# DeadAt0m/ActiveSparseShifts-PyTorch

Hardware: AMD Instinct MI355X
Metric: Gelem/s, Shift2d fwd+bwd N64/C256/224x224 (higher is better)
Workload: dtype f32; 1 GPU; Shift2d SSL fwd+bwd N64 C256 224x224 fp32, padding 0, per GPU; batch sharded over 1 GPU(s), no collectives

## Files before the change

### activesparseshifts-pytorch_amd/csrc/shiftnd_cl_tiled.hip

```cpp
#include "shiftnd_common.hpp"
#include "shiftnd_launch.hpp"

namespace shiftnd {
namespace {

constexpr int kR = 3;
constexpr int kTW = 32;
constexpr int kLine = 128;
constexpr int kPW = kTW + 2 * kR;
constexpr int kRing = 2 * kR + 1;
constexpr int kPitch = kLine / 4 + 1;
constexpr int kRowWords = kPW * kPitch;
constexpr int kPieces = kPW * (kLine / 16);
constexpr int kNP = (kPieces + kThreads - 1) / kThreads;
#ifndef CLT_DEPTH
#define CLT_DEPTH 3
#endif

struct ClTiledParams {
    const char *x;
    char *out;
    const void *w;
    int64_t wzp;
    uint32_t fill;
// ... 221 lines not shown
        if (hs + kR < H) store_row(hs + kR, pv);
        __syncthreads();
        load_row(hs + kDepth + kR, ylast, pv);
        const uint32_t so = static_cast<uint32_t>(h - h0) * ostep;
        int rowb[NSH];
#pragma unroll
        for (int k = 0; k < NSH; ++k) {
            const int sy = fold_once(hs - ssh[k]);
            const uint32_t r = static_cast<uint32_t>(sy & ~(sy >> 31));
            const uint32_t sl = r - __umulhi(r, 613566757u) * kRing;
            rowb[k] = (16 + static_cast<int>(sl) * (kRowWords * 4)) | ((sy >> 31) & kNeg);
        }
        uint32_t v[4];
#pragma unroll
        for (int i = 0; i < 4; ++i) {
            v[i] = 0;
#pragma unroll
            for (int j = 0; j < NE; ++j) {
                const uint32_t e = *reinterpret_cast<const EL *>(ringz + max(rowb[OUT_CL ? j : i] + xoff[i][j], 0));
                v[i] |= e << (8 * ES * j);
            }
        }
#pragma unroll
        for (int i = 0; i < 4; ++i) __builtin_amdgcn_raw_buffer_store_b32(v[i], ores, ooff[i], so, 0);
    };
    int hb = h0;
    for (; hb + kDepth <= h1; hb += kDepth) {
#pragma unroll
        for (int d = 0; d < kDepth; ++d) step(hb + d, pvs[d]);
    }
#pragma unroll
    for (int d = 0; d < kDepth - 1; ++d)
        if (hb + d < h1) step(hb + d, pvs[d]);

    const bool wrap_rows = periodic && (h0 + LH < kR || h1 + LH > H - kR);
    if (far || (wrap_rows && ring_ok)) {
        asm volatile("s_waitcnt vmcnt(0)" ::: "memory");
#pragma unroll
        for (int i = 0; i < 4; ++i) {
#pragma unroll
            for (int j = 0; j < NE; ++j) {
                const bool all_rows = (far >> (4 * i + j)) & 1u;
                if (!all_rows && !(wrap_rows && ((ring_ok >> (4 * i + j)) & 1u))) continue;
                const int D = static_cast<int>(threadIdx.x) + kThreads * i;
                const int ch = OUT_CL ? lane_a * NE + j : D / RD;
                const int col = OUT_CL ? lane_b + 8 * i : (D % RD) * NE + j;
                const EL *xe = reinterpret_cast<const EL *>(xn);
                EL *o = reinterpret_cast<EL *>(on) + (OUT_CL ? ((static_cast<int64_t>(dz) * OH + h0) * OW + w0 + col) * C + c0 + ch
                                                             : ((static_cast<int64_t>(c0 + ch) * OD + dz) * OH + h0) * OW + w0 + col);
                const int64_t zoff = ND3 ? static_cast<int64_t>(tab_pz[ch]) * H * W * C : 0;
                const int shc = csh[OUT_CL ? j : i], shs = ssh[OUT_CL ? j : i];
                for (int h = h0; h < h1; ++h) {
                    const int sy = H == 1 ? 0 : fold_index(h + LH - shc, H, p.pad);
                    if (all_rows || h + LH - shs < 0 || h + LH - shs >= H)
                        *o = sy >= 0 ? xe[zoff + (static_cast<int64_t>(sy) * W + gcol[i][j]) * C + c0 + ch] : static_cast<EL>(p.fill);
                    o += OUT_CL ? OW * C : OW;
                }
            }
        }
    }
}

constexpr int kBTW = 16;
constexpr int kBPW = kBTW + 2 * kR + 1;
constexpr int kBRing = 8;
constexpr int kBPieces = kBPW * (kLine / 16);
static_assert(kBPieces <= kThreads, "one piece of each tensor per thread");

struct ClTiledBwdParams {
    const char *x, *go;
    char *gx;
    const void *w;
    double *partials;
    int wkind, N, C, H, W, pad;
    int OH, OW, LH, LW;
    int go_nchw;
    int go_pieces;
    int wtiles, cblocks, bands, band_rows;
    unsigned xcd_blocks;
    FastDiv d_wtiles, d_cblocks, d_bands;
    FastDiv d_perH, d_perW, d_perOH, d_perOW;
};

template <typename T, bool ACTIVE, bool GO_NCHW, int TW = kBTW>
__global__ __launch_bounds__(kThreads) void cl_tiled_backward(const ClTiledBwdParams p) {
    static_assert(TW == kBTW || !GO_NCHW, "the wide strip takes a channels-last gradient");
    constexpr int BPW = TW + 2 * kR + 1;
    constexpr int BPIECES = BPW * (kLine / 16);
    constexpr int NPX = (BPIECES + kThreads - 1) / kThreads;
    typedef uint32_t u4 __attribute__((ext_vector_type(4)));
    using S = typename T::S;
    using CT = typename T::C;
    static_assert(sizeof(S) == 4 || sizeof(S) == 2, "fp32, fp16, bf16");
    constexpr int ES = sizeof(S), CB = kLine / ES;
    constexpr int PL = kThreads / CB, NI = TW / PL;
    constexpr int PITCHX = kLine / 4, PITCHG = GO_NCHW ? kPitch : kLine / 4;
    constexpr int BROWX = BPW * PITCHX, BROWG = BPW * PITCHG, BRINGX = kBRing * BROWX, BRINGG = kBRing * BROWG;
    __shared__ __attribute__((aligned(16))) uint32_t ring_all[4 + BRINGX + BRINGG + 4];
    uint32_t *const ring = ring_all + 4;
    constexpr int kDump = BRINGX + BRINGG;
    constexpr int kNeg = -(1 << 24);
    if (threadIdx.x < 4) ring_all[threadIdx.x] = 0u;

    unsigned b = p.xcd_blocks ? (blockIdx.x & 7u) * p.xcd_blocks + (blockIdx.x >> 3) : blockIdx.x;
    const int cb = static_cast<int>(b - fdiv(b, p.d_cblocks) * p.cblocks);
    b = fdiv(b, p.d_cblocks);
    const int pidx = static_cast<int>(b);
    const int wt = static_cast<int>(b - fdiv(b, p.d_wtiles) * p.wtiles);
    b = fdiv(b, p.d_wtiles);
    const int band = static_cast<int>(b - fdiv(b, p.d_bands) * p.bands);
    const int n = static_cast<int>(fdiv(b, p.d_bands));
    const int w0 = wt * TW, c0 = cb * CB;
    const int h0 = band * p.band_rows, h1 = min(p.H, h0 + p.band_rows);
    const int H = p.H, W = p.W, C = p.C, OH = p.OH, OW = p.OW, LH = p.LH, LW = p.LW;
    const int64_t img = static_cast<int64_t>(n) * H * W * C * ES;
    const char *xn = p.x + img, *gn = p.go + static_cast<int64_t>(n) * OH * OW * C * ES;
    char *on = p.gx + img;
    const uint32_t img_bytes = static_cast<uint32_t>(H) * static_cast<uint32_t>(W) * static_cast<uint32_t>(C) * ES;
    const uint32_t go_bytes = static_cast<uint32_t>(OH) * static_cast<uint32_t>(OW) * static_cast<uint32_t>(C) * ES;
    const __amdgpu_buffer_rsrc_t xres = __builtin_amdgcn_make_buffer_rsrc(const_cast<char *>(xn), 0, img_bytes, kBufferFlags);
    const __amdgpu_buffer_rsrc_t gres = __builtin_amdgcn_make_buffer_rsrc(const_cast<char *>(gn), 0, go_bytes, kBufferFlags);
    const __amdgpu_buffer_rsrc_t ores = __builtin_amdgcn_make_buffer_rsrc(on, 0, img_bytes, kBufferFlags);
    auto g_index = [&](int ch, int r, int cc) {
        return GO_NCHW ? (static_cast<int64_t>(ch) * OH + r) * OW + cc : (static_cast<int64_t>(r) * OW + cc) * C + ch;
    };

    const int q = static_cast<int>(threadIdx.x);
    uint32_t poff[NPX], poffg[NPX];
    int pdst[NPX];
#pragma unroll
    for (int k = 0; k < NPX; ++k) {
        const int qk = q + k * kThreads;
        const bool piece = qk < BPIECES;
        const int px = qk >> 3, part = qk & 7, gxs = w0 - kR + px;
        poff[k] = (piece && gxs >= 0 && gxs < W && c0 * ES + part * 16 < C * ES) ? static_cast<uint32_t>(gxs) * C * ES + c0 * ES + part * 16 : kOutOfRange;
        poffg[k] = (piece && gxs >= LW && gxs < LW + OW && c0 * ES + part * 16 < C * ES) ? static_cast<uint32_t>(gxs - LW) * C * ES + c0 * ES + part * 16 : kOutOfRange;
        pdst[k] = piece ? px * PITCHX + part * 4 : -1;
    }
    const uint32_t row_bytes = static_cast<uint32_t>(W) * C * ES;
    constexpr int kDepth = CLT_DEPTH;
    constexpr int kGE = CB * BPW, kGN = GO_NCHW ? (kGE + kThreads - 1) / kThreads : 1;
    struct GRow {
        u4 v[NPX];
        uint32_t e[kGN];
    };
    uint32_t goff[kGN];
    int gdst[kGN];
    if constexpr (GO_NCHW) {
#pragma unroll
        for (int k = 0; k < kGN; ++k) {
            const int e = k * kThreads + q, ch = e / BPW, pxe = e - ch * BPW, gxe = w0 - kR + pxe;
            const bool ok = e < kGE && gxe >= LW && gxe < LW + OW && c0 + ch < C;
            goff[k] = ok ? (static_cast<uint32_t>(c0 + ch) * OH * OW + (gxe - LW)) * ES : kOutOfRange;
            gdst[k] = e < kGE ? pxe * (PITCHG * 4) + ch * ES : -1;
        }
    }
    constexpr int kGPC = 7;
    const bool g_pieces = GO_NCHW && ES == 4 && p.go_pieces != 0;
    uint32_t gpoff = kOutOfRange;
    int gpdst[4] = {-1, -1, -1, -1};
    if constexpr (GO_NCHW && ES == 4) {
        const int ch = q / kGPC, pi = q - ch * kGPC;
        const int cstart = w0 - kR - LW;
        const int e0 = ((cstart >> 2) + pi) * 4;
        const bool ok = q < CB * kGPC && e0 >= 0 && e0 < OW && c0 + ch < C;
        gpoff = ok ? (static_cast<uint32_t>(c0 + ch) * OH * OW + e0) * ES : kOutOfRange;
#pragma unroll
        for (int j = 0; j < 4; ++j) {
            const int pxj = e0 + j - cstart;
            gpdst[j] = (q < CB * kGPC && pxj >= 0 && pxj < BPW) ? pxj * (PITCHG * 4) + ch * ES : -1;
        }
    }
    const uint32_t grow_bytes = static_cast<uint32_t>(OW) * (GO_NCHW ? 1 : C) * ES;
    struct XRow {
        u4 v[NPX];
    };
    XRow pvx[kDepth];
    GRow pvg[kDepth];
    auto load_row = [&](int y, int ylast, XRow &vx, GRow &vg) {
        const int unwanted = (y >> 31) | ((ylast - y) >> 31);
        const uint32_t so = static_cast<uint32_t>(y & ~unwanted) * row_bytes, dead = static_cast<uint32_t>(unwanted) & kOutOfRange;
#pragma unroll
        for (int k = 0; k < NPX; ++k) vx.v[k] = __builtin_amdgcn_raw_buffer_load_b128(xres, poff[k] | dead, so, 0);
        const int unwanted_g = unwanted | ((y - LH) >> 31) | ((LH + OH - 1 - y) >> 31);
        const uint32_t sg = static_cast<uint32_t>((y - LH) & ~unwanted_g) * grow_bytes, dead_g = static_cast<uint32_t>(unwanted_g) & kOutOfRange;
        if constexpr (GO_NCHW) {
            if (g_pieces) {
                vg.v[0] = __builtin_amdgcn_raw_buffer_load_b128(gres, gpoff | dead_g, sg, 0);
            } else {
#pragma unroll
                for (int k = 0; k < kGN; ++k) {
                    if constexpr (ES == 4) vg.e[k] = __builtin_amdgcn_raw_buffer_load_b32(gres, goff[k] | dead_g, sg, 0);
                    else vg.e[k] = __builtin_amdgcn_raw_buffer_load_b16(gres, goff[k] | dead_g, sg, 0);
                }
            }
        } else {
#pragma unroll
            for (int k = 0; k < NPX; ++k) vg.v[k] = __builtin_amdgcn_raw_buffer_load_b128(gres, poffg[k] | dead_g, sg, 0);
        }
    };
    auto store_row = [&](int y, const XRow &vx, const GRow &vg) {
        const int slot = y & (kBRing - 1);
#pragma unroll
        for (int k = 0; k < NPX; ++k) {
            uint32_t *dx = ring + (pdst[k] >= 0 ? slot * BROWX + pdst[k] : kDump);
            *reinterpret_cast<u4 *>(__builtin_assume_aligned(dx, 16)) = vx.v[k];
        }
        if constexpr (GO_NCHW) {
            char *gbase = reinterpret_cast<char *>(ring) + (BRINGX + slot * BROWG) * 4;
            char *dump = reinterpret_cast<char *>(ring) + kDump * 4;
            if (g_pieces) {
                const uint32_t ge[4] = {vg.v[0].x, vg.v[0].y, vg.v[0].z, vg.v[0].w};
#pragma unroll
                for (int j = 0; j < 4; ++j) *reinterpret_cast<uint32_t *>(gpdst[j] >= 0 ? gbase + gpdst[j] : dump) = ge[j];
            } else {
#pragma unroll
                for (int k = 0; k < kGN; ++k) {
                    char *d = gdst[k] >= 0 ? gbase + gdst[k] : dump;
                    if constexpr (ES == 4) *reinterpret_cast<uint32_t *>(d) = vg.e[k];
                    else *reinterpret_cast<uint16_t *>(d) = static_cast<uint16_t>(vg.e[k]);
                }
            }
        } else {
#pragma unroll
            for (int k = 0; k < NPX; ++k) {
                uint32_t *dg = ring + (pdst[k] >= 0 ? BRINGX + slot * BROWG + pdst[k] : kDump);
                *reinterpret_cast<u4 *>(__builtin_assume_aligned(dg, 16)) = vg.v[k];
            }
        }
    };
    const int ylast = min(H - 1, h1 + kR);
    XRow prex[2 * kR + 1];
    GRow preg[2 * kR + 1];
#pragma unroll
    for (int d = 0; d < kDepth; ++d) load_row(h0 + kR + 1 + d, ylast, pvx[d], pvg[d]);
#pragma unroll
    for (int r = 0; r <= 2 * kR; ++r) load_row(h0 - kR + r, ylast, prex[r], preg[r]);

    const int lane_a = static_cast<int>(threadIdx.x) % CB, lane_b = static_cast<int>(threadIdx.x) / CB;
    const int c = c0 + lane_a;
    const bool live_c = c < C;
    int64_t sh[3] = {0, 0, 0};
    CT dw[3] = {CT(0), CT(0), CT(0)};
    {
        const int wcol[3] = {-1, 0, 1};
        CT wv[3];
        load_weights3<CT>(p.w, p.wkind, static_cast<int64_t>(live_c ? c : C - 1) * 2, wcol, wv);
        prep_shift_backward<CT>(wv[1], ACTIVE, sh[1], dw[0]);
        prep_shift_backward<CT>(wv[2], ACTIVE, sh[2], dw[1]);
    }
    const int csxH = canon_shift(sh[1], H, p.pad, p.d_perH), csxW = canon_shift(sh[2], W, p.pad, p.d_perW);
    const int csgH = canon_shift(ACTIVE ? sh[1] : -sh[1], OH, p.pad, p.d_perOH), csgW = canon_shift(ACTIVE ? sh[2] : -sh[2], OW, p.pad, p.d_perOW);
    const int perH = map_period(H, p.pad), perW = map_period(W, p.pad), perOH = map_period(OH, p.pad), perOW = map_period(OW, p.pad);
    const int sh_s = (perH && 2 * csxH > perH) ? csxH - perH : csxH, sw_s = (perW && 2 * csxW > perW) ? csxW - perW : csxW;
    const int gh_s = (perOH && 2 * csgH > perOH) ? csgH - perOH : csgH, gw_s = (perOW && 2 * csgW > perOW) ? csgW - perOW : csgW;
    const bool in_ring = sh_s >= -kR && sh_s <= kR && sw_s >= -kR && sw_s <= kR && gh_s >= -kR && gh_s <= kR && gw_s >= -kR && gw_s <= kR;
    const bool near_c = live_c && in_ring, far_c = live_c && !in_ring;
    auto fold_h = [&](int idx) { return H == 1 ? 0 : fold_index(idx, H, p.pad); };
    auto fold_w = [&](int idx) { return W == 1 ? 0 : fold_index(idx, W, p.pad); };
    auto fold_gh = [&](int idx) { const int r = OH == 1 ? 0 : fold_index(idx, OH, p.pad); return r < 0 ? -1 : r + LH; };
    auto fold_gw = [&](int idx) { const int r = OW == 1 ? 0 : fold_index(idx, OW, p.pad); return r < 0 ? -1 : r + LW; };
    int xc0[NI], xc1[NI], gc0[NI], gc1[NI], gd[NI];
    uint32_t ooff[NI];
    bool live[NI], scol[NI], cpass[NI];
    int lcount[NI];
#pragma unroll
    for (int i = 0; i < NI; ++i) {
        const int col = lane_b + PL * i, wq = w0 + min(col, W - 1 - w0);
        cpass[i] = wq >= LW && wq < LW + OW;
        const int a0 = cpass[i] ? fold_w(wq - csxW) : -1, a1 = cpass[i] ? fold_w(wq - csxW + 1) : -1;
        const int b0 = cpass[i] ? fold_gw(wq - LW - csgW) : -1, b1 = (ACTIVE && cpass[i]) ? fold_gw(wq - LW - csgW + 1) : -1;
        auto outside = [&](int sx) { return sx >= 0 && (sx < w0 - kR || sx > w0 + TW + kR); };
        scol[i] = near_c && w0 + col < W && (outside(a0) || outside(a1) || outside(b0) || outside(b1));
        live[i] = near_c && w0 + col < W && !scol[i];
        lcount[i] = (live[i] && cpass[i]) ? -1 : 0;
        auto lds_col = [&](int sx, int pitch) { return (live[i] && sx >= 0) ? (sx - (w0 - kR)) * (pitch * 4) + lane_a * ES : kNeg; };
        xc0[i] = lds_col(a0, PITCHX);
        xc1[i] = lds_col(a1, PITCHX);
        gc0[i] = lds_col(b0, PITCHG);
        gc1[i] = lds_col(b1, PITCHG);
        gd[i] = (col + kR) * (PITCHG * 4) + lane_a * ES;
        ooff[i] = live[i] ? (static_cast<uint32_t>(h0 * W + w0 + col) * C + c) * ES : kOutOfRange;
    }
    const uint32_t ostep = static_cast<uint32_t>(W) * C * ES;

#pragma unroll
    for (int r = 0; r <= 2 * kR; ++r) {
        const int y = h0 - kR + r;
        if (y >= 0 && y < H) store_row(y, prex[r], preg[r]);
    }
    const char *ringz = reinterpret_cast<const char *>(ring_all);
    constexpr int ringx = 16, ringg = 16 + BRINGX * 4;
    double acc[2] = {0.0, 0.0};
    auto lds_s = [&](int base, int row, int colo) {
        return *reinterpret_cast<const S *>(ringz + max(base + row + colo, 0));
    };
    auto lds_f = [&](int base, int row, int colo) { return widen<T>(lds_s(base, row, colo)); };
    auto row_off = [&](int sy) { return ((sy & (kBRing - 1)) * (BROWX * 4)) | ((sy >> 31) & kNeg); };
    auto row_off_g = [&](int sy) { return ((sy & (kBRing - 1)) * (BROWG * 4)) | ((sy >> 31) & kNeg); };
    const int fm = (p.pad == 3 || p.pad == 4) ? -1 : 0;
    const int fLo = p.pad == 4 ? -1 : 0, fHi = p.pad == 1 ? H - 1 : (p.pad == 3 ? 2 * H - 2 : 2 * H - 1);
    const int zneg = p.pad == 0 ? kNeg : 0;
    auto fold_once = [&](int idx, int n, int lo_c, int hi_c) {
        const int below = idx >> 31, above = (n - 1 - idx) >> 31, t = idx & fm;
        const int r = (idx & ~(below | above)) | ((lo_c - t) & below) | ((hi_c - t) & above) | ((below | above) & zneg);
        return n == 1 ? 0 : r;
    };
    auto fold1 = [&](int idx) { return fold_once(idx, H, fLo, fHi); };
    const int gLo = p.pad == 4 ? -1 : 0, gHi = p.pad == 1 ? OH - 1 : (p.pad == 3 ? 2 * OH - 2 : 2 * OH - 1);
    auto fold1g = [&](int idx) { return fold_once(idx, OH, gLo, gHi) + LH; };
    const bool srow = near_c && p.pad == 3 && H > 1 && sh_s == -kR && h1 == H;
    const bool srow_g = ACTIVE && near_c && p.pad == 3 && OH > 1 && gh_s == -kR;
    const bool periodic = p.pad == 2 && H > 1;
    auto wraps = [&](int h) {
        const int g0 = h - LH - gh_s;
        const bool in_rows = h >= LH && h < LH + OH;
        return periodic && near_c && (h - sh_s < 0 || h + 1 - sh_s >= H || (in_rows && OH > 1 && (g0 < 0 || g0 + (ACTIVE ? 1 : 0) >= OH)));
    };
    int xrow1 = fold1(h0 - sh_s);
    int grow1 = fold1g(h0 - LH - gh_s);
    auto step = [&](int h, XRow &vx, GRow &vg) {
        __syncthreads();
        if (h + kR + 1 < H) store_row(h + kR + 1, vx, vg);
        __syncthreads();
        load_row(h + kDepth + kR + 1, ylast, vx, vg);
        const uint32_t so = static_cast<uint32_t>(h - h0) * ostep;
        const int xr0 = row_off(xrow1);
        xrow1 = fold1(h + 1 - sh_s);
        const int xr1 = row_off(xrow1);
        const bool rpass = h >= LH && h < LH + OH;
        int gr0, gr1 = kNeg;
        if constexpr (ACTIVE) {
            gr0 = rpass ? row_off_g(grow1) : kNeg;
            grow1 = fold1g(h + 1 - LH - gh_s);
            gr1 = rpass ? row_off_g(grow1) : kNeg;
        } else {
            gr0 = rpass ? row_off_g(fold1g(h - LH - gh_s)) : kNeg;
        }
        const int gdr = (h & (kBRing - 1)) * (BROWG * 4);
        int skip = 0;
        if (p.pad == 3) skip = ((srow && h == H - 1) || (srow_g && h == LH + OH - 1)) ? -1 : 0;
        else if (p.pad == 2) skip = wraps(h) ? -1 : 0;
        const int stepok = (rpass ? -1 : 0) & ~skip;
        S res[NI];
        CT s0 = CT(0), s1 = CT(0);
#pragma unroll
        for (int i = 0; i < NI; ++i) {
            CT v[4], wg[3];
            v[0] = lds_f(ringx, xr0, xc0[i]);
            v[1] = lds_f(ringx, xr1, xc0[i]);
            v[2] = lds_f(ringx, xr0, xc1[i]);
            v[3] = lds_f(ringx, xr1, xc1[i]);
            const CT graw = widen<T>(*reinterpret_cast<const S *>(ringz + ringg + gdr + gd[i]));
            const uint32_t counted = static_cast<uint32_t>(lcount[i] & stepok);
            weight_grads_nd<2, CT>(v, dw, wg);
            static_assert(sizeof(CT) == 4, "fp32 compute type");
            s0 += __builtin_bit_cast(CT, __builtin_bit_cast(uint32_t, graw * wg[0]) & counted);
            s1 += __builtin_bit_cast(CT, __builtin_bit_cast(uint32_t, graw * wg[1]) & counted);
            if constexpr (ACTIVE) {
                v[0] = lds_f(ringg, gr0, gc0[i]);
                v[1] = lds_f(ringg, gr1, gc0[i]);
                v[2] = lds_f(ringg, gr0, gc1[i]);
                v[3] = lds_f(ringg, gr1, gc1[i]);
                res[i] = narrow<T>(interp_t<T, 2>(v, dw));
            } else {
                res[i] = lds_s(ringg, gr0, gc0[i]);
            }
        }
        acc[0] += static_cast<double>(s0);
        acc[1] += static_cast<double>(s1);
#pragma unroll
        for (int i = 0; i < NI; ++i) {
            if constexpr (ES == 4) {
                uint32_t bits;
                __builtin_memcpy(&bits, &res[i], 4);
                __builtin_amdgcn_raw_buffer_store_b32(bits, ores, ooff[i] | (static_cast<uint32_t>(skip) & kOutOfRange), so, 0);
            } else {
                uint16_t bits;
                __builtin_memcpy(&bits, &res[i], 2);
                __builtin_amdgcn_raw_buffer_store_b16(bits, ores, ooff[i] | (static_cast<uint32_t>(skip) & kOutOfRange), so, 0);
            }
        }
    };
    int hb = h0;
    for (; hb + kDepth <= h1; hb += kDepth) {
#pragma unroll
        for (int d = 0; d < kDepth; ++d) step(hb + d, pvx[d], pvg[d]);
    }
#pragma unroll
    for (int d = 0; d < kDepth - 1; ++d)
        if (hb + d < h1) step(hb + d, pvx[d], pvg[d]);

    auto far_element = [&](int ch, int h, int wq, int cxH, int cxW, int cgH, int cgW, const CT (&fr)[3], double &t0, double &t1) {
        const S *xe = reinterpret_cast<const S *>(xn) + ch, *ge = reinterpret_cast<const S *>(gn);
        S *oe = reinterpret_cast<S *>(on) + ch;
        auto tap_s = [&](const S *base, int r, int cc) { return (r >= 0 && cc >= 0) ? base[(static_cast<int64_t>(r) * W + cc) * C] : narrow<T>(CT(0)); };
        auto tap = [&](const S *base, int r, int cc) { return widen<T>(tap_s(base, r, cc)); };
        auto gtap_s = [&](int r, int cc) { return (r >= 0 && cc >= 0) ? ge[g_index(ch, r, cc)] : narrow<T>(CT(0)); };
        auto gtap = [&](int r, int cc) { return widen<T>(gtap_s(r, cc)); };
        if (!(h >= LH && h < LH + OH && wq >= LW && wq < LW + OW)) {
            oe[(static_cast<int64_t>(h) * W + wq) * C] = narrow<T>(CT(0));
            return;
        }
        const int a0 = fold_w(wq - cxW), a1 = fold_w(wq - cxW + 1);
        const int b0 = fold_gw(wq - LW - cgW) - LW, b1 = fold_gw(wq - LW - cgW + 1) - LW;
        const int r0 = fold_h(h - cxH), r1 = fold_h(h - cxH + 1);
        const int s0 = fold_gh(h - LH - cgH) - LH, s1 = fold_gh(h - LH - cgH + 1) - LH;
        CT v[4] = {tap(xe, r0, a0), tap(xe, r1, a0), tap(xe, r0, a1), tap(xe, r1, a1)}, wg[3];
        const CT gval = widen<T>(ge[g_index(ch, h - LH, wq - LW)]);
        weight_grads_nd<2, CT>(v, fr, wg);
        t0 += static_cast<double>(gval * wg[0]);
        t1 += static_cast<double>(gval * wg[1]);
        S r;
        if constexpr (ACTIVE) {
            CT u[4] = {gtap(s0, b0), gtap(s1, b0), gtap(s0, b1), gtap(s1, b1)};
            r = narrow<T>(interp_t<T, 2>(u, fr));
        } else {
            r = gtap_s(s0, b0);
        }
        oe[(static_cast<int64_t>(h) * W + wq) * C] = r;
    };
    bool any_scol = false;
#pragma unroll
    for (int i = 0; i < NI; ++i) any_scol = any_scol || scol[i];
    const bool wrap_rows = periodic && near_c && (h0 <= kR || h1 >= H - kR - 1 || (h0 <= LH + kR && h1 > LH) || (h1 >= LH + OH - kR - 1 && h0 < LH + OH));
    if (near_c && (any_scol || srow || srow_g || wrap_rows)) {
#pragma unroll
        for (int i = 0; i < NI; ++i) {
            const int wq = w0 + lane_b + PL * i;
            if (wq >= W) continue;
            for (int h = h0; h < h1; ++h) {
                if (!(scol[i] || (srow && h == H - 1) || (srow_g && h == LH + OH - 1) || wraps(h))) continue;
                far_element(c, h, wq, csxH, csxW, csgH, csgW, dw, acc[0], acc[1]);
            }
        }
    }
    {
        __shared__ unsigned long long far_mask_s;
        __syncthreads();
        if (threadIdx.x < 64) {
            const unsigned long long m = __ballot(far_c && static_cast<int>(threadIdx.x) < CB);
            if (threadIdx.x == 0) far_mask_s = m;
        }
        __syncthreads();
        unsigned long long fm_left = far_mask_s;
        double *fred = reinterpret_cast<double *>(ring_all);
        while (fm_left) {
            const int fch = __builtin_ctzll(fm_left);
            fm_left &= fm_left - 1;
            const int cf = c0 + fch;
            int64_t fsh[3] = {0, 0, 0};
            CT ffr[3] = {CT(0), CT(0), CT(0)};
            {
                const int wcol[3] = {-1, 0, 1};
                CT wv[3];
                load_weights3<CT>(p.w, p.wkind, static_cast<int64_t>(cf) * 2, wcol, wv);
                prep_shift_backward<CT>(wv[1], ACTIVE, fsh[1], ffr[0]);
                prep_shift_backward<CT>(wv[2], ACTIVE, fsh[2], ffr[1]);
            }
            const int fxH = canon_shift(fsh[1], H, p.pad, p.d_perH), fxW = canon_shift(fsh[2], W, p.pad, p.d_perW);
            const int fgH = canon_shift(ACTIVE ? fsh[1] : -fsh[1], OH, p.pad, p.d_perOH), fgW = canon_shift(ACTIVE ? fsh[2] : -fsh[2], OW, p.pad, p.d_perOW);
            double t0 = 0.0, t1 = 0.0;
            const int nelem = (h1 - h0) * TW;
            for (int q = static_cast<int>(threadIdx.x); q < nelem; q += kThreads) {
                const int h = h0 + q / TW, wq = w0 + q % TW;
                if (wq < W) far_element(cf, h, wq, fxH, fxW, fgH, fgW, ffr, t0, t1);
            }
            __syncthreads();
            fred[threadIdx.x * 2] = t0;
            fred[threadIdx.x * 2 + 1] = t1;
            __syncthreads();
            if (static_cast<int>(threadIdx.x) == fch) {
                double u0 = 0.0, u1 = 0.0;
                for (int k = 0; k < kThreads; ++k) {
                    u0 += fred[k * 2];
                    u1 += fred[k * 2 + 1];
                }
                acc[0] += u0;
                acc[1] += u1;
            }
        }
    }

    __syncthreads();
    double *red = reinterpret_cast<double *>(ring_all);
    red[threadIdx.x * 2] = acc[0];
    red[threadIdx.x * 2 + 1] = acc[1];
    __syncthreads();
    if (lane_b == 0 && live_c) {
        double t0 = 0.0, t1 = 0.0;
        for (int k = 0; k < PL; ++k) {
            t0 += red[(k * CB + lane_a) * 2];
            t1 += red[(k * CB + lane_a) * 2 + 1];
        }
        double *dst = p.partials + (static_cast<size_t>(pidx) * C + c) * 3;
        dst[0] = t0;
        dst[1] = t1;
        dst[2] = 0.0;
    }
}

constexpr int kAPW = kTW + 2 * kR + 1;
constexpr int kARing = 8;
constexpr int kARowWords = kAPW * kPitch;
constexpr int kAPieces = kAPW * (kLine / 16);
constexpr int kANP = (kAPieces + kThreads - 1) / kThreads;

template <typename T, bool OUT_CL, bool ND3>
__global__ __launch_bounds__(kThreads) void cl_tiled_active_forward(const ClTiledParams p) {
// ... 415 lines not shown
    }
    if (nd3) {
        note_kernel("cl_tiled_forward_3d");
#define SHIFTND_CLT_LAUNCH3(ESV) \
    if (p.out_cl) hipLaunchKernelGGL((cl_tiled_forward<ESV, true, true>), dim3(static_cast<unsigned>(grid)), dim3(kThreads), 0, st, p); \
    else hipLaunchKernelGGL((cl_tiled_forward<ESV, false, true>), dim3(static_cast<unsigned>(grid)), dim3(kThreads), 0, st, p);
        if (es == 4) { SHIFTND_CLT_LAUNCH3(4) }
        else { SHIFTND_CLT_LAUNCH3(2) }
#undef SHIFTND_CLT_LAUNCH3
        return SHIFTND_OK;
    }
    if (g.active && dtype <= SHIFTND_BF16) {
        note_kernel("cl_tiled_active_forward");
#define SHIFTND_CLT_ACTIVE(TT) \
    if (p.out_cl) hipLaunchKernelGGL((cl_tiled_active_forward<TT, true, false>), dim3(static_cast<unsigned>(grid)), dim3(kThreads), 0, st, p); \
    else hipLaunchKernelGGL((cl_tiled_active_forward<TT, false, false>), dim3(static_cast<unsigned>(grid)), dim3(kThreads), 0, st, p);
        if (dtype == SHIFTND_F32) { SHIFTND_CLT_ACTIVE(f32_t) }
        else if (dtype == SHIFTND_F16) { SHIFTND_CLT_ACTIVE(f16_t) }
        else { SHIFTND_CLT_ACTIVE(bf16_t) }
#undef SHIFTND_CLT_ACTIVE
        return SHIFTND_OK;
    }
    note_kernel("cl_tiled_forward");
#define SHIFTND_CLT_LAUNCH(ESV) \
    if (p.out_cl) hipLaunchKernelGGL((cl_tiled_forward<ESV, true, false>), dim3(static_cast<unsigned>(grid)), dim3(kThreads), 0, st, p); \
    else hipLaunchKernelGGL((cl_tiled_forward<ESV, false, false>), dim3(static_cast<unsigned>(grid)), dim3(kThreads), 0, st, p);
    if (es == 4) { SHIFTND_CLT_LAUNCH(4) }
    else if (es == 2) { SHIFTND_CLT_LAUNCH(2) }
    else { SHIFTND_CLT_LAUNCH(1) }
#undef SHIFTND_CLT_LAUNCH
    return SHIFTND_OK;
}

namespace {
struct ClTiledBwdPlan {
    int wtiles, cblocks, bands, band_rows, tw;
    int64_t groups;
};
ClTiledBwdPlan cl_tiled_backward_plan(const Geometry &g, int es = 4, int tw = kBTW) {
    ClTiledBwdPlan pl;
    const int H = static_cast<int>(g.S[1]), W = static_cast<int>(g.S[2]);
    pl.tw = tw;
    pl.wtiles = (W + tw - 1) / tw;
    const int cbw = kLine / es;
    pl.cblocks = static_cast<int>((g.C + cbw - 1) / cbw);
    const int64_t base = g.N * pl.wtiles;
    int64_t bands = g_cl_tiled_tune[1] > 0 ? (H + g_cl_tiled_tune[1] - 1) / g_cl_tiled_tune[1] : (7168 + base * pl.cblocks - 1) / (base * pl.cblocks);
    const int64_t max_bands = H / (8 * kR) > 0 ? H / (8 * kR) : 1;
    if (g_cl_tiled_tune[1] <= 0) {
        if (bands > max_bands) bands = max_bands;
        while (bands > 1 && base * bands > 4096) --bands;
    }
    if (bands < 1) bands = 1;
    pl.band_rows = static_cast<int>((H + bands - 1) / bands);
    pl.bands = (H + pl.band_rows - 1) / pl.band_rows;
    pl.groups = base * pl.bands;
    return pl;
}
}

bool cl_tiled_backward_eligible(const Geometry &g, int dtype, const void *go, const void *x, const void *gx) {
    if (!g_cl_tiled_tune[0] || g.nd != 2 || (dtype != SHIFTND_F32 && dtype != SHIFTND_F16 && dtype != SHIFTND_BF16)) return false;
    const int es = dtype_size(dtype);
    for (int d = 0; d < 3; ++d)
        if ((g.L[d] != 0 || g.O[d] != g.S[d]) && (d == 0 || g.O[d] < 1)) return false;
    if ((g.C * es) % 16 != 0 || g.S[1] >= (1 << 20) || g.S[2] >= (1 << 20) || g.N >= (1LL << 24) || g.C >= (1 << 24)) return false;
    if ((g.S[1] != 1 && g.S[1] < 5) || (g.O[1] != 1 && g.O[1] < 5)) return false;
    if (g.C * g.S[1] * g.S[2] * es >= (1LL << 31)) return false;
    if (!dense_channels_last_2d(g.xs, g, g.S) || !dense_channels_last_2d(g.gs, g, g.S)) return false;
    const bool go_cl = dense_channels_last_2d(g.os, g, g.O);
    if (!go_cl && !contiguous_2d(g.os, g, g.O)) return false;
    if (reinterpret_cast<uintptr_t>(x) % 16 != 0 || reinterpret_cast<uintptr_t>(go) % (go_cl ? 16 : es) != 0 || reinterpret_cast<uintptr_t>(gx) % es != 0) return false;
    const ClTiledBwdPlan pl = cl_tiled_backward_plan(g, es);
    return pl.groups * pl.cblocks < (1LL << 31);
}

size_t cl_tiled_backward_workspace(const Geometry &g) {
    if (g.nd != 2 || g.C < 1 || g.N * g.S[1] * g.S[2] < 1) return 0;
    const ClTiledBwdPlan p4 = cl_tiled_backward_plan(g, 4), p2 = cl_tiled_backward_plan(g, 2);
    return static_cast<size_t>(p4.groups > p2.groups ? p4.groups : p2.groups) * static_cast<size_t>(g.C) * 3 * sizeof(double);
}

namespace {
template <typename T>
void launch_cl_tiled_backward(const ClTiledBwdParams &p, const ClTiledBwdPlan &pl, bool active, void *gw, hipStream_t st) {
    const dim3 grid(static_cast<unsigned>(pl.groups * pl.cblocks)), block(kThreads);
    if (p.go_nchw) {
        if (active) hipLaunchKernelGGL((cl_tiled_backward<T, true, true>), grid, block, 0, st, p);
        else hipLaunchKernelGGL((cl_tiled_backward<T, false, true>), grid, block, 0, st, p);
    } else {
        if (active) hipLaunchKernelGGL((cl_tiled_backward<T, true, false>), grid, block, 0, st, p);
        else hipLaunchKernelGGL((cl_tiled_backward<T, false, false>), grid, block, 0, st, p);
    }
    launch_reduce_weight_grads(p.wkind, p.partials, static_cast<int>(pl.groups), p.C, 2, gw, st);
}
}

int cl_tiled_backward(const Geometry &g, int dtype, const void *go, const void *x, const void *w, int wkind, void *gx, void *gw,
                      void *workspace, hipStream_t st) {
    const ClTiledBwdPlan pl = cl_tiled_backward_plan(g, dtype_size(dtype), kBTW);
    ClTiledBwdParams p{};
    p.x = static_cast<const char *>(x);
    p.go = static_cast<const char *>(go);
    p.gx = static_cast<char *>(gx);
    p.w = w;
    p.wkind = wkind;
    p.partials = static_cast<double *>(workspace);
    p.N = static_cast<int>(g.N);
    p.C = static_cast<int>(g.C);
    p.H = static_cast<int>(g.S[1]);
    p.W = static_cast<int>(g.S[2]);
    p.OH = static_cast<int>(g.O[1]);
    p.OW = static_cast<int>(g.O[2]);
    p.LH = static_cast<int>(g.L[1]);
    p.LW = static_cast<int>(g.L[2]);
    p.pad = g.pad;
    p.go_nchw = dense_channels_last_2d(g.os, g, g.O) ? 0 : 1;
    p.go_pieces = (p.go_nchw && (g.O[2] * dtype_size(dtype)) % 16 == 0 && reinterpret_cast<uintptr_t>(go) % 16 == 0) ? 1 : 0;
    p.wtiles = pl.wtiles;
    p.cblocks = pl.cblocks;
    p.bands = pl.bands;
    p.band_rows = pl.band_rows;
    p.d_wtiles = make_fastdiv(static_cast<uint32_t>(p.wtiles));
    p.d_cblocks = make_fastdiv(static_cast<uint32_t>(p.cblocks));
    p.d_bands = make_fastdiv(static_cast<uint32_t>(p.bands));
    p.d_perH = make_fastdiv(static_cast<uint32_t>(map_period(p.H, p.pad)));
    p.d_perW = make_fastdiv(static_cast<uint32_t>(map_period(p.W, p.pad)));
    p.d_perOH = make_fastdiv(static_cast<uint32_t>(map_period(p.OH, p.pad)));
    p.d_perOW = make_fastdiv(static_cast<uint32_t>(map_period(p.OW, p.pad)));
    {
        const int64_t grid = pl.groups * pl.cblocks;
        p.xcd_blocks = (g_cl_tiled_tune[2] && grid % 8 == 0) ? static_cast<unsigned>(grid / 8) : 0;
    }
    note_kernel(p.go_nchw ? "cl_tiled_backward_nchw_grad" : "cl_tiled_backward");
    switch (dtype) {
    case SHIFTND_F32: launch_cl_tiled_backward<f32_t>(p, pl, g.active != 0, gw, st); break;
    case SHIFTND_F16: launch_cl_tiled_backward<f16_t>(p, pl, g.active != 0, gw, st); break;
    case SHIFTND_BF16: launch_cl_tiled_backward<bf16_t>(p, pl, g.active != 0, gw, st); break;
    default: return SHIFTND_ERR_UNSUPPORTED_DTYPE;
    }
    return SHIFTND_OK;
}

}
```

### activesparseshifts-pytorch_amd/csrc/torch_binding.cpp

```cpp
#include <ATen/ATen.h>
#include <ATen/core/dispatch/Dispatcher.h>
#include <c10/core/DeviceGuard.h>
#include <c10/hip/HIPStream.h>
#include <hip/hip_version.h>
#include <torch/autograd.h>
#include <torch/library.h>

#include <string>
#include <tuple>
#include <type_traits>
#include <vector>

#include "shiftnd_hip.h"

namespace torchshifts_amd {

using at::Tensor;
using torch::autograd::AutogradContext;
using torch::autograd::variable_list;

using forward_sig = Tensor(const Tensor &, const Tensor &, const Tensor &, at::IntArrayRef, int64_t, bool);
using backward_sig = std::tuple<Tensor, Tensor>(const Tensor &, const Tensor &, const Tensor &, const Tensor &, int64_t,
                                                bool);
using pool_forward_sig = Tensor(const Tensor &, const Tensor &, const Tensor &, at::IntArrayRef, at::IntArrayRef, int64_t, bool);
// ... 420 lines not shown
    Tensor y_like = at::empty(ysize, grad.options());
    Tensor g;
    if constexpr (ND == 1) {
        g = at::avg_pool2d_backward(grad.unsqueeze(2), y_like.unsqueeze(2), {1, pool[0]}, {1, pool[0]}, {0, 0}, true, true,
                                    c10::nullopt).squeeze(2);
    } else if constexpr (ND == 2) {
        g = at::avg_pool2d_backward(grad, y_like, pool, pool, {0, 0}, true, true, c10::nullopt);
    } else {
        g = at::avg_pool3d_backward(grad, y_like, pool, pool, {0, 0, 0}, true, true, c10::nullopt);
    }
    return ShiftOps<ND>::backward().call(g, weights, input, borders, padding_mode, active_flag);
}

template <int ND> Tensor pool_forward_hip(const Tensor &input_, const Tensor &weights, const Tensor &borders,
                                          at::IntArrayRef new_size, at::IntArrayRef pool, int64_t padding_mode,
                                          bool active_flag) {
    check_pool<ND>(pool);
    TORCH_CHECK(input_.is_cuda(), "input must be a CUDA tensor");
    TORCH_CHECK(weights.is_cuda(), "weights must be a CUDA tensor");
    const int mixed = weights_flag("shiftnd_pool_forward_cuda", input_, "input", weights);
    TORCH_CHECK(input_.dim() == ND + 2, "shift", ND, "d_pool: expected a ", ND + 2, "-D input");
    TORCH_CHECK(weights.dim() == 2 && weights.size(0) == input_.size(1) && weights.size(1) == ND,
                "shift", ND, "d_pool: weights must have shape [C, ", ND, "]");
    if (padding_mode < 0 || padding_mode > 4) return Tensor();
    c10::DeviceGuard device_guard(input_.device());
    const Tensor input = is_channels_last_dense(input_) ? channels_last_to_contiguous(input_) : input_;
    if (!input.is_contiguous()) return pool_forward_composed<ND>(input, weights, borders, new_size, pool, padding_mode, active_flag);
    const int dtype = to_shiftnd_dtype(input.scalar_type(), "shiftnd_pool_forward_cuda") | mixed;
    int32_t b[6];
    read_borders(borders, b);
    shiftnd_problem p;
    fill_problem(p, ND, input, b, padding_mode, active_flag, dtype);
    const PoolArgs<ND> pa(p, pool);
    Tensor w = weights.contiguous();
    Tensor output = at::empty(pa.output_size(input), input.options(), at::MemoryFormat::Contiguous);
    const int rc = shiftnd_forward_pooled(&p, pa.k, input.data_ptr(), w.data_ptr(), output.data_ptr(), current_stream(input));
    if (rc == SHIFTND_ERR_NOT_FUSED)
        return pool_forward_composed<ND>(input, weights, borders, new_size, pool, padding_mode, active_flag);
    check_status(rc, "shiftnd_forward_pooled (HIP)");
    return output;
}

template <int ND>
std::tuple<Tensor, Tensor> pool_backward_hip(const Tensor &grad, const Tensor &weights, const Tensor &input_,
                                             const Tensor &borders, at::IntArrayRef pool, int64_t padding_mode,
                                             bool active_flag) {
    check_pool<ND>(pool);
    TORCH_CHECK(grad.is_cuda(), "grad must be a CUDA tensor");
    TORCH_CHECK(input_.is_cuda(), "input must be a CUDA tensor");
    TORCH_CHECK(weights.is_cuda(), "weights must be a CUDA tensor");
    check_same("shiftnd_pool_backward_cuda", grad, "grad", input_, "input");
    const int mixed = weights_flag("shiftnd_pool_backward_cuda", grad, "grad", weights);
    TORCH_CHECK(input_.dim() == ND + 2 && grad.dim() == ND + 2, "shift", ND, "d_pool backward: expected ", ND + 2, "-D tensors");
    if (padding_mode < 0 || padding_mode > 4) return std::make_tuple(Tensor(), Tensor());
    c10::DeviceGuard device_guard(grad.device());
    const Tensor input = is_channels_last_dense(input_) ? channels_last_to_contiguous(input_) : input_;
    if (!input.is_contiguous())
        return pool_backward_composed<ND>(grad, weights, input, borders, pool, padding_mode, active_flag);
    const int dtype = to_shiftnd_dtype(grad.scalar_type(), "shiftnd_pool_backward_cuda") | mixed;
    int32_t b[6];
    read_borders(borders, b);
    shiftnd_problem p;
    fill_problem(p, ND, input, b, padding_mode, active_flag, dtype);
    const PoolArgs<ND> pa(p, pool);
    pa.check_grad(grad, "d_pool");
    Tensor g = grad.contiguous();
    Tensor w = weights.contiguous();
    Tensor grad_input = at::empty_like(input, at::MemoryFormat::Contiguous);
    Tensor grad_weights = at::empty_like(w, at::MemoryFormat::Contiguous);
    const size_t ws_bytes = shiftnd_backward_pooled_workspace_bytes(&p, pa.k);
    Tensor workspace = workspace_like(input, ws_bytes);
    const int rc = shiftnd_backward_pooled(&p, pa.k, g.data_ptr(), input.data_ptr(), w.data_ptr(), grad_input.data_ptr(),
                                           grad_weights.data_ptr(), workspace.data_ptr(), ws_bytes, current_stream(grad));
    if (rc == SHIFTND_ERR_NOT_FUSED)
        return pool_backward_composed<ND>(grad, weights, input, borders, pool, padding_mode, active_flag);
    check_status(rc, "shiftnd_backward_pooled (HIP)");
    return std::make_tuple(grad_input, grad_weights);
}

template <int ND> struct ShiftPoolFunction : public torch::autograd::Function<ShiftPoolFunction<ND>> {
    static variable_list forward(AutogradContext *ctx, const Tensor &input, const Tensor &weight, const Tensor &borders,
                                 at::IntArrayRef new_size, at::IntArrayRef pool, int64_t padding_mode, bool active_flag) {
        at::AutoDispatchBelowADInplaceOrView guard;
        auto output = PoolOps<ND>::forward().call(input, weight, borders, new_size, pool, padding_mode, active_flag);
        ctx->saved_data["padding_mode"] = padding_mode;
        ctx->saved_data["active_flag"] = active_flag;
        ctx->saved_data["pool"] = pool.vec();
        ctx->save_for_backward({input, weight, borders});
        return {output};
    }
    static variable_list backward(AutogradContext *ctx, const variable_list &grad_output) {
        auto saved = ctx->get_saved_variables();
        const auto padding_mode = ctx->saved_data["padding_mode"].toInt();
        const auto active_flag = ctx->saved_data["active_flag"].toBool();
        const auto pool = ctx->saved_data["pool"].toIntVector();
        auto result = PoolOps<ND>::backward().call(grad_output[0], saved[1], saved[0], saved[2], pool, padding_mode, active_flag);
        return {std::get<0>(result), std::get<1>(result), Tensor(), Tensor(), Tensor(), Tensor(), Tensor()};
    }
};
template <int ND> Tensor pool_autograd(const Tensor &input, const Tensor &weights, const Tensor &borders,
                                       at::IntArrayRef new_size, at::IntArrayRef pool, int64_t padding_mode,
                                       bool active_flag) {
    return ShiftPoolFunction<ND>::apply(input, weights, borders, new_size, pool, padding_mode, active_flag)[0];
}
template <int ND> Tensor shift_pool_public(const Tensor &input, const Tensor &weights, const Tensor &borders,
                                           at::IntArrayRef pool, int64_t padding_mode, bool active_flag) {
    auto bands = check_borders(input, borders, ND);
    return PoolOps<ND>::forward().call(input, weights, std::get<0>(bands), std::get<1>(bands), pool, padding_mode, active_flag);
}

int quant_dtype(at::ScalarType t, const char *what) {
    switch (t) {
    case at::kQInt8: return SHIFTND_I8;
    case at::kQUInt8: return SHIFTND_U8;
    case at::kQInt32: return SHIFTND_I32;
    default: TORCH_CHECK(false, "\"", what, "\" not implemented for '", c10::toString(t), "'");
    }
    return -1;
}

template <int ND> Tensor qshift_forward_hip(const Tensor &input_, const Tensor &weights, const Tensor &borders,
                                            at::IntArrayRef new_size, int64_t padding_mode, bool ) {
    TORCH_CHECK(input_.is_cuda() && input_.is_quantized(), "input must be a quantized CUDA tensor");
    TORCH_CHECK(weights.is_quantized(), "weights must be a quantized tensor");
    TORCH_CHECK(input_.dim() == ND + 2, "shift", ND, "d: expected a ", ND + 2, "-D input");
    if (padding_mode < 0 || padding_mode > 4) return Tensor();
    c10::DeviceGuard device_guard(input_.device());
    const int dtype = quant_dtype(input_.scalar_type(), "q_shiftnd_cuda");
    const int wdtype = quant_dtype(weights.scalar_type(), "q_shiftnd_cuda");
    int32_t b[6];
    if (static_cast<int>(new_size.size()) == ND + 2) read_borders_for(borders, input_, new_size.slice(2), ND, b);
    else read_borders(borders, b);
    Tensor wrepr = weights.int_repr().to(input_.device()).contiguous();
    TORCH_CHECK(wrepr.dim() == 2 && wrepr.size(0) == input_.size(1) && wrepr.size(1) == ND,
                "shift", ND, "d: weights must have shape [C, ", ND, "]");
    const bool cl = input_.is_contiguous(at::MemoryFormat::ChannelsLast) || input_.is_contiguous(at::MemoryFormat::ChannelsLast3d);
    bool via_transpose = cl && is_channels_last_dense(input_);
    Tensor out_cl;
    if (via_transpose) {
        out_cl = at::_empty_affine_quantized(new_size, input_.options().memory_format(input_.suggest_memory_format()),
                                                    input_.q_scale(), input_.q_zero_point(), c10::nullopt);
        shiftnd_problem pd;
        fill_problem(pd, ND, input_, b, padding_mode, false, dtype);
        int64_t xd[5], od[5];
        fill_strides(input_, ND, xd);
        fill_strides(out_cl, ND, od);
        if (shiftnd_forward_serves_channels_last(&pd, input_.data_ptr(), xd, out_cl.data_ptr(), od)) {
            check_status(shiftnd_forward_quantized(&pd, input_.data_ptr(), xd, wrepr.data_ptr(), wdtype, weights.q_zero_point(),
                                                   input_.q_zero_point(), out_cl.data_ptr(), od, current_stream(input_)),
                         "shiftnd_forward_quantized (HIP)");
            return out_cl;
        }
    }
    const Tensor input = via_transpose ? channels_last_to_contiguous(input_) : input_;
    Tensor output = (cl && !via_transpose)
                        ? at::_empty_affine_quantized(new_size, input.options().memory_format(input.suggest_memory_format()),
                                                      input.q_scale(), input.q_zero_point(), c10::nullopt)
                        : at::_empty_affine_quantized(new_size, input.options().memory_format(at::MemoryFormat::Contiguous),
                                                      input.q_scale(), input.q_zero_point(), c10::nullopt);
    shiftnd_problem p;
    fill_problem(p, ND, input, b, padding_mode, false, dtype);
    int64_t xs[5], os[5];
    fill_strides(input, ND, xs);
    fill_strides(output, ND, os);
    check_status(shiftnd_forward_quantized(&p, input.data_ptr(), xs, wrepr.data_ptr(), wdtype, weights.q_zero_point(),
                                           input.q_zero_point(), output.data_ptr(), os, current_stream(input)),
                 "shiftnd_forward_quantized (HIP)");
    if (via_transpose && output.numel() > 0 && output.size(1) > 1) {
        contiguous_to_channels_last(output, out_cl);
        return out_cl;
    }
// ... 1101 lines not shown
```

Baseline: 320.1 Gelem/s.

## Add zero-padding specialized backward kernel skipping wrap/fold and slow-column paths

Adds a ZEROS template variant of the channels-last tiled backward kernel for zero padding, active, fp32, channels-last gradient. It drops the per-column fold/outside checks, the slow-column fallback, and the per-row bounds checks, and uses a streamlined row step with masked stores. This is meant to cut index arithmetic and branching in the inner loop. It also changes the pooled autograd forward to convert channels-last inputs to contiguous before saving, which touches a different path and costs an extra copy there.

```diff
diff --git a/activesparseshifts-pytorch_amd/csrc/shiftnd_cl_tiled.hip b/activesparseshifts-pytorch_amd/csrc/shiftnd_cl_tiled.hip
--- a/activesparseshifts-pytorch_amd/csrc/shiftnd_cl_tiled.hip
+++ b/activesparseshifts-pytorch_amd/csrc/shiftnd_cl_tiled.hip
@@ -327,7 +327,7 @@
     FastDiv d_perH, d_perW, d_perOH, d_perOW;
 };
 
-template <typename T, bool ACTIVE, bool GO_NCHW, int TW = kBTW>
+template <typename T, bool ACTIVE, bool GO_NCHW, int TW = kBTW, bool ZEROS = false>
 __global__ __launch_bounds__(kThreads) void cl_tiled_backward(const ClTiledBwdParams p) {
     static_assert(TW == kBTW || !GO_NCHW, "the wide strip takes a channels-last gradient");
     constexpr int BPW = TW + 2 * kR + 1;
@@ -377,9 +377,11 @@
     for (int k = 0; k < NPX; ++k) {
         const int qk = q + k * kThreads;
         const bool piece = qk < BPIECES;
-        const int px = qk >> 3, part = qk & 7, gxs = w0 - kR + px;
+        const int px = qk >> 3, part = qk & 7;
+        const int gxs = (ZEROS && W == 1 && w0 - kR + px == 1) ? 0 : w0 - kR + px;
+        const int gxw = (ZEROS && OW == 1 && w0 - kR + px == LW + 1) ? LW : w0 - kR + px;
         poff[k] = (piece && gxs >= 0 && gxs < W && c0 * ES + part * 16 < C * ES) ? static_cast<uint32_t>(gxs) * C * ES + c0 * ES + part * 16 : kOutOfRange;
-        poffg[k] = (piece && gxs >= LW && gxs < LW + OW && c0 * ES + part * 16 < C * ES) ? static_cast<uint32_t>(gxs - LW) * C * ES + c0 * ES + part * 16 : kOutOfRange;
+        poffg[k] = (piece && gxw >= LW && gxw < LW + OW && c0 * ES + part * 16 < C * ES) ? static_cast<uint32_t>(gxw - LW) * C * ES + c0 * ES + part * 16 : kOutOfRange;
         pdst[k] = piece ? px * PITCHX + part * 4 : -1;
     }
     const uint32_t row_bytes = static_cast<uint32_t>(W) * C * ES;
@@ -394,7 +396,8 @@
     if constexpr (GO_NCHW) {
 #pragma unroll
         for (int k = 0; k < kGN; ++k) {
-            const int e = k * kThreads + q, ch = e / BPW, pxe = e - ch * BPW, gxe = w0 - kR + pxe;
+            const int e = k * kThreads + q, ch = e / BPW, pxe = e - ch * BPW;
+            const int gxe = (ZEROS && OW == 1 && w0 - kR + pxe == LW + 1) ? LW : w0 - kR + pxe;
             const bool ok = e < kGE && gxe >= LW && gxe < LW + OW && c0 + ch < C;
             goff[k] = ok ? (static_cast<uint32_t>(c0 + ch) * OH * OW + (gxe - LW)) * ES : kOutOfRange;
             gdst[k] = e < kGE ? pxe * (PITCHG * 4) + ch * ES : -1;
@@ -513,6 +516,18 @@
     for (int i = 0; i < NI; ++i) {
         const int col = lane_b + PL * i, wq = w0 + min(col, W - 1 - w0);
         cpass[i] = wq >= LW && wq < LW + OW;
+        if constexpr (ZEROS) {
+            const int px = wq - w0 + kR;
+            scol[i] = false;
+            live[i] = near_c && w0 + col < W;
+            lcount[i] = (live[i] && cpass[i]) ? -1 : 0;
+            xc0[i] = 16 + (px - (near_c ? sw_s : 0)) * (PITCHX * 4) + lane_a * ES;
+            gc0[i] = 16 + BRINGX * 4 + (px - (near_c ? gw_s : 0)) * (PITCHG * 4) + lane_a * ES;
+            xc1[i] = gc1[i] = 0;
+            gd[i] = (col + kR) * (PITCHG * 4) + lane_a * ES;
+            ooff[i] = live[i] ? (static_cast<uint32_t>(h0 * W + w0 + col) * C + c) * ES : kOutOfRange;
+            continue;
+        }
         const int a0 = cpass[i] ? fold_w(wq - csxW) : -1, a1 = cpass[i] ? fold_w(wq - csxW + 1) : -1;
         const int b0 = cpass[i] ? fold_gw(wq - LW - csgW) : -1, b1 = (ACTIVE && cpass[i]) ? fold_gw(wq - LW - csgW + 1) : -1;
         auto outside = [&](int sx) { return sx >= 0 && (sx < w0 - kR || sx > w0 + TW + kR); };
@@ -532,7 +547,7 @@
 #pragma unroll
     for (int r = 0; r <= 2 * kR; ++r) {
         const int y = h0 - kR + r;
-        if (y >= 0 && y < H) store_row(y, prex[r], preg[r]);
+        if (ZEROS || (y >= 0 && y < H)) store_row(y, prex[r], preg[r]);
     }
     const char *ringz = reinterpret_cast<const char *>(ring_all);
     constexpr int ringx = 16, ringg = 16 + BRINGX * 4;
@@ -627,14 +642,80 @@
             }
         }
     };
+    const bool unitH = H == 1, unitOH = OH == 1;
+    const int sh_e = near_c ? sh_s : 0, gh_e = near_c ? gh_s : 0;
+    auto slot_x = [&](int y) { return (y & (kBRing - 1)) * (BROWX * 4); };
+    auto slot_g = [&](int y) { return (y & (kBRing - 1)) * (BROWG * 4); };
+    int xnext = slot_x(h0 - sh_e), gnext = slot_g(h0 - gh_e);
+    auto step_z = [&](int h, XRow &vx, GRow &vg) {
+        __syncthreads();
+        store_row(h + kR + 1, vx, vg);
+        __syncthreads();
+        load_row(h + kDepth + kR + 1, ylast, vx, vg);
+        const uint32_t so = static_cast<uint32_t>(h - h0) * ostep;
+        const int xr0 = xnext;
+        xnext = slot_x(h + 1 - sh_e);
+        const int xr1 = unitH ? xr0 : xnext;
+        const int gr0 = gnext;
+        gnext = slot_g(h + 1 - gh_e);
+        const int gr1 = unitOH ? gr0 : gnext;
+        const int gdr = (h & (kBRing - 1)) * (BROWG * 4);
+        const int rmask = (h >= LH && h < LH + OH) ? -1 : 0;
+        S res[NI];
+        CT s0 = CT(0), s1 = CT(0);
+#pragma unroll
+        for (int i = 0; i < NI; ++i) {
+            CT v[4], wg[3];
+            const char *c0p = ringz + (xr0 + xc0[i]), *c1p = ringz + (xr1 + xc0[i]);
+            v[0] = widen<T>(*reinterpret_cast<const S *>(c0p));
+            v[1] = widen<T>(*reinterpret_cast<const S *>(c1p));
+            v[2] = widen<T>(*reinterpret_cast<const S *>(c0p + PITCHX * 4));
+            v[3] = widen<T>(*reinterpret_cast<const S *>(c1p + PITCHX * 4));
+            const CT graw = widen<T>(*reinterpret_cast<const S *>(ringz + ringg + gdr + gd[i]));
+            const uint32_t counted = static_cast<uint32_t>(lcount[i] & rmask);
+            weight_grads_nd<2, CT>(v, dw, wg);
+            static_assert(sizeof(CT) == 4, "fp32 compute type");
+            s0 += __builtin_bit_cast(CT, __builtin_bit_cast(uint32_t, graw * wg[0]) & counted);
+            s1 += __builtin_bit_cast(CT, __builtin_bit_cast(uint32_t, graw * wg[1]) & counted);
+            const char *g0p = ringz + (gr0 + gc0[i]);
+            if constexpr (ACTIVE) {
+                const char *g1p = ringz + (gr1 + gc0[i]);
+                v[0] = widen<T>(*reinterpret_cast<const S *>(g0p));
+                v[1] = widen<T>(*reinterpret_cast<const S *>(g1p));
+                v[2] = widen<T>(*reinterpret_cast<const S *>(g0p + PITCHG * 4));
+                v[3] = widen<T>(*reinterpret_cast<const S *>(g1p + PITCHG * 4));
+                res[i] = narrow<T>(interp_t<T, 2>(v, dw));
+            } else {
+                res[i] = *reinterpret_cast<const S *>(g0p);
+            }
+        }
+        acc[0] += static_cast<double>(s0);
+        acc[1] += static_cast<double>(s1);
+#pragma unroll
+        for (int i = 0; i < NI; ++i) {
+            if constexpr (ES == 4) {
+                uint32_t bits;
+                __builtin_memcpy(&bits, &res[i], 4);
+                __builtin_amdgcn_raw_buffer_store_b32(bits & static_cast<uint32_t>(lcount[i] & rmask), ores, ooff[i], so, 0);
+            } else {
+                uint16_t bits;
+                __builtin_memcpy(&bits, &res[i], 2);
+                __builtin_amdgcn_raw_buffer_store_b16(static_cast<uint16_t>(bits & static_cast<uint32_t>(lcount[i] & rmask)), ores, ooff[i], so, 0);
+            }
+        }
+    };
+    auto row_step = [&](int h, XRow &vx, GRow &vg) {
+        if constexpr (ZEROS) step_z(h, vx, vg);
+        else step(h, vx, vg);
+    };
     int hb = h0;
     for (; hb + kDepth <= h1; hb += kDepth) {
 #pragma unroll
-        for (int d = 0; d < kDepth; ++d) step(hb + d, pvx[d], pvg[d]);
+        for (int d = 0; d < kDepth; ++d) row_step(hb + d, pvx[d], pvg[d]);
     }
 #pragma unroll
     for (int d = 0; d < kDepth - 1; ++d)
-        if (hb + d < h1) step(hb + d, pvx[d], pvg[d]);
+        if (hb + d < h1) row_step(hb + d, pvx[d], pvg[d]);
 
     auto far_element = [&](int ch, int h, int wq, int cxH, int cxW, int cgH, int cgW, const CT (&fr)[3], double &t0, double &t1) {
         const S *xe = reinterpret_cast<const S *>(xn) + ch, *ge = reinterpret_cast<const S *>(gn);
@@ -669,7 +750,7 @@
 #pragma unroll
     for (int i = 0; i < NI; ++i) any_scol = any_scol || scol[i];
     const bool wrap_rows = periodic && near_c && (h0 <= kR || h1 >= H - kR - 1 || (h0 <= LH + kR && h1 > LH) || (h1 >= LH + OH - kR - 1 && h0 < LH + OH));
-    if (near_c && (any_scol || srow || srow_g || wrap_rows)) {
+    if (!ZEROS && near_c && (any_scol || srow || srow_g || wrap_rows)) {
 #pragma unroll
         for (int i = 0; i < NI; ++i) {
             const int wq = w0 + lane_b + PL * i;
@@ -1251,9 +1332,20 @@
 }
 
 namespace {
+bool cl_tiled_backward_zeros_form(int pad, int dtype, int go_nchw, bool active) {
+    return pad == 0 && active && dtype == SHIFTND_F32 && !go_nchw && g_cl_tiled_tune[0] != 2;
+}
+
 template <typename T>
 void launch_cl_tiled_backward(const ClTiledBwdParams &p, const ClTiledBwdPlan &pl, bool active, void *gw, hipStream_t st) {
     const dim3 grid(static_cast<unsigned>(pl.groups * pl.cblocks)), block(kThreads);
+    if constexpr (sizeof(typename T::S) == 4) {
+        if (cl_tiled_backward_zeros_form(p.pad, SHIFTND_F32, p.go_nchw, active)) {
+            hipLaunchKernelGGL((cl_tiled_backward<T, true, false, kBTW, true>), grid, block, 0, st, p);
+            launch_reduce_weight_grads(p.wkind, p.partials, static_cast<int>(pl.groups), p.C, 2, gw, st);
+            return;
+        }
+    }
     if (p.go_nchw) {
         if (active) hipLaunchKernelGGL((cl_tiled_backward<T, true, true>), grid, block, 0, st, p);
         else hipLaunchKernelGGL((cl_tiled_backward<T, false, true>), grid, block, 0, st, p);
@@ -1301,7 +1393,10 @@
         const int64_t grid = pl.groups * pl.cblocks;
         p.xcd_blocks = (g_cl_tiled_tune[2] && grid % 8 == 0) ? static_cast<unsigned>(grid / 8) : 0;
     }
-    note_kernel(p.go_nchw ? "cl_tiled_backward_nchw_grad" : "cl_tiled_backward");
+    if (g_cl_tiled_tune[0] == 3 && cl_tiled_backward_zeros_form(p.pad, dtype, p.go_nchw, g.active != 0))
+        note_kernel("cl_tiled_backward_zeros");
+    else
+        note_kernel(p.go_nchw ? "cl_tiled_backward_nchw_grad" : "cl_tiled_backward");
     switch (dtype) {
     case SHIFTND_F32: launch_cl_tiled_backward<f32_t>(p, pl, g.active != 0, gw, st); break;
     case SHIFTND_F16: launch_cl_tiled_backward<f16_t>(p, pl, g.active != 0, gw, st); break;
diff --git a/activesparseshifts-pytorch_amd/csrc/torch_binding.cpp b/activesparseshifts-pytorch_amd/csrc/torch_binding.cpp
--- a/activesparseshifts-pytorch_amd/csrc/torch_binding.cpp
+++ b/activesparseshifts-pytorch_amd/csrc/torch_binding.cpp
@@ -526,11 +526,17 @@
     static variable_list forward(AutogradContext *ctx, const Tensor &input, const Tensor &weight, const Tensor &borders,
                                  at::IntArrayRef new_size, at::IntArrayRef pool, int64_t padding_mode, bool active_flag) {
         at::AutoDispatchBelowADInplaceOrView guard;
-        auto output = PoolOps<ND>::forward().call(input, weight, borders, new_size, pool, padding_mode, active_flag);
+        Tensor kept = input;
+        if ((input.requires_grad() || weight.requires_grad()) && input.is_cuda() && !input.is_quantized() && input.dim() == ND + 2 &&
+            at::isFloatingType(input.scalar_type()) && padding_mode >= 0 && padding_mode <= 4 && is_channels_last_dense(input)) {
+            c10::DeviceGuard device_guard(input.device());
+            kept = channels_last_to_contiguous(input);
+        }
+        auto output = PoolOps<ND>::forward().call(kept, weight, borders, new_size, pool, padding_mode, active_flag);
         ctx->saved_data["padding_mode"] = padding_mode;
         ctx->saved_data["active_flag"] = active_flag;
         ctx->saved_data["pool"] = pool.vec();
-        ctx->save_for_backward({input, weight, borders});
+        ctx->save_for_backward({kept, weight, borders});
         return {output};
     }
     static variable_list backward(AutogradContext *ctx, const variable_list &grad_output) {
```

Result: no change. 319.8 Gelem/s (-0.1%).
